# LuizGuzzo/Monocular_Depth_Estimation

Measured on AMD Instinct MI355X. Metric: training images/sec at 640x480 bs=32/GPU (GuideDepth, SSIM+0.1*L1, Adam), higher is better.
Workload: dtype fp32; 1 GPU; GuideDepth (DDRNet-23-slim + 3 guided upsampling blocks) train step, BASELINE cfg2, BN in train mode; global_batch=32, per_gpu_batch=32, resolution=640x480, parallelism=dp1

## Files before the change

### include/mde_abi.h

```cpp
#ifndef MDE_ABI_H
#define MDE_ABI_H

#include <stddef.h>
#include <stdint.h>

#ifdef __cplusplus
extern "C" {
#endif

#define MDE_ABI_VERSION 1

#define MDE_F32 0
#define MDE_BF16 1

#define MDE_OK 0
#define MDE_ERR_INVALID_ARG (-1)
#define MDE_ERR_UNSUPPORTED (-2)

int mde_abi_version(void);
const char* mde_status_string(int status);


int mde_bilinear_fwd(const void* x, void* y, int64_t n, int64_t c, int64_t hi,
                     int64_t wi, int64_t ho, int64_t wo, float scale_h,
// ... 234 lines not shown
int mde_conv3x3_wgrad(const void* gy, const void* x, float* gweight, int64_t n, int64_t cin,
                      int64_t cout, int64_t h, int64_t w, void* workspace, int dtype,
                      void* stream);

int mde_conv3x3s2_supported(int64_t cin, int64_t cout, int dtype);
size_t mde_conv3x3s2_wgrad_workspace(int64_t n, int64_t cin, int64_t cout, int64_t h, int64_t w,
                                     int dtype);
int mde_conv3x3s2_wgrad(const void* gy, const void* x, float* gweight, int64_t n, int64_t cin,
                        int64_t cout, int64_t h, int64_t w, void* workspace, int dtype,
                        void* stream);

size_t mde_dwconv_workspace(int64_t n, int64_t c, int64_t h, int64_t w, int64_t k,
                            int64_t stride, int64_t pad);
int mde_dwconv_fwd(const void* x, const float* weight, void* y, int64_t n, int64_t c,
                   int64_t h, int64_t w, int64_t k, int64_t stride, int64_t pad, int dtype,
                   void* stream);
int mde_dwconv_bwd(const void* gy, const void* x, const float* weight, void* gx,
                   float* gweight, int64_t n, int64_t c, int64_t h, int64_t w, int64_t k,
                   int64_t stride, int64_t pad, void* workspace, int dtype, void* stream);

size_t mde_layernorm_workspace(int64_t rows, int64_t c);
int mde_layernorm_fwd(const void* x, const float* gamma, const float* beta, void* y,
                      float* mean, float* rstd, int64_t rows, int64_t c, float eps, int dtype,
                      void* stream);
int mde_layernorm_bwd(const void* gy, const void* x, const float* gamma, const float* mean,
                      const float* rstd, void* gx, float* ggamma, float* gbeta, int64_t rows,
                      int64_t c, void* workspace, int dtype, void* stream);
int mde_layernorm_add_fwd(const void* x, const void* r, const float* gamma, const float* beta,
                          void* sum, void* y, float* mean, float* rstd, int64_t rows, int64_t c,
                          float eps, int dtype, void* stream);
int mde_layernorm_bwd_res(const void* gy, const void* x, const void* gres, const float* gamma,
                          const float* mean, const float* rstd, void* gx, float* ggamma,
                          float* gbeta, int64_t rows, int64_t c, void* workspace, int dtype,
                          void* stream);

int mde_transpose(const void* x, void* y, int64_t batch, int64_t m, int64_t n, int dtype,
                  void* stream);

int mde_nyu_augment(const void* image, const void* depth, const int32_t* flags, float* image_out,
                    float* depth_out, int64_t n, int64_t h, int64_t w, int64_t dh, int64_t dw,
                    int depth_bits, void* stream);

size_t mde_eval_workspace(int64_t n, int64_t h, int64_t w);
int mde_eval_sums(const void* pred, const void* gt, int64_t n, int64_t h, int64_t w,
                  float min_depth, float max_depth, int mode, const int32_t* crop,
                  void* workspace, double* sums, int dtype, void* stream);

int mde_conv3x3_guide_bf16_stats_blocks(int64_t n, int64_t cout, int64_t h, int64_t w);
int mde_conv3x3_guide_bf16_fwd(const float* x, const float* weight, void* y, float* stats,
                               int64_t n, int64_t cout, int64_t h, int64_t w, void* stream);

int mde_conv1x1_supported(int64_t cin, int64_t cout, int64_t h, int64_t w, int stride,
                          int dtype);
int mde_conv1x1_fwd(const void* x, const float* weight, void* y, int64_t n, int64_t cin,
                    int64_t cout, int64_t h, int64_t w, int stride, int dtype, void* stream);
int mde_conv1x1_bwd_data(const void* gy, const float* weight, void* gx, int64_t n, int64_t cin,
                         int64_t cout, int64_t h, int64_t w, int stride, int dtype,
                         void* stream);
size_t mde_conv1x1_wgrad_workspace(int64_t n, int64_t cin, int64_t cout, int64_t h, int64_t w,
                                   int stride, int dtype);
int mde_conv1x1_wgrad(const void* gy, const void* x, float* gweight, int64_t n, int64_t cin,
                      int64_t cout, int64_t h, int64_t w, int stride, void* workspace, int dtype,
                      void* stream);

int mde_conv3x3s2_fwd_supported(int64_t cin, int64_t cout, int64_t h, int64_t w, int dtype);
int mde_conv3x3s2_dgrad_supported(int64_t cin, int64_t cout, int64_t h, int64_t w, int dtype);
int mde_conv3x3s2_fwd(const void* x, const float* weight, void* y, int64_t n, int64_t cin,
                      int64_t cout, int64_t h, int64_t w, int dtype, void* stream);
int mde_conv3x3s2_bwd_data(const void* gy, const float* weight, void* gx, int64_t n, int64_t cin,
                           int64_t cout, int64_t h, int64_t w, int dtype, void* stream);

int mde_conv3x3_wide_supported(int64_t cin, int64_t cout, int64_t h, int64_t w, int pass,
                               int dtype);
int mde_conv3x3_wide_fwd(const void* x, const float* weight, void* y, int64_t n, int64_t cin,
                         int64_t cout, int64_t h, int64_t w, int dtype, void* stream);
int mde_conv3x3_wide_bwd_data(const void* gy, const float* weight, void* gx, int64_t n,
                              int64_t cin, int64_t cout, int64_t h, int64_t w, int dtype,
                              void* stream);

int mde_conv3x3s2_fwd_instance(int64_t n, int64_t cin, int64_t cout, int64_t h, int64_t w);
int mde_conv3x3s2_dgrad_instance(int64_t n, int64_t cin, int64_t cout, int64_t h, int64_t w);
int mde_conv3x3_wide_instance(int64_t n, int64_t cin, int64_t cout, int64_t h, int64_t w,
                              int pass);
int mde_conv3x3s2_instance_count(int which);

int mde_wino_mode(int mode);
int mde_wino_supported(int64_t cin, int64_t cout, int64_t h, int64_t w, int dtype);
size_t mde_wino_weight_bytes(int64_t cin, int64_t cout);
int mde_wino_weight(const float* weight, float* u, int64_t cin, int64_t cout, int flip,
                    void* stream);
int mde_wino_weight2(const float* weight, float* u, float* u_flip, int64_t cin, int64_t cout,
                     void* stream);
int mde_wino_conv(const float* x, const float* u, float* y, int64_t n, int64_t cin, int64_t cout,
                  int64_t h, int64_t w, int pass, int dtype, void* stream);
int mde_wino_conv_acc(const float* x, const float* u, const float* add, float* y, int64_t n,
                      int64_t cin, int64_t cout, int64_t h, int64_t w, int pass, int dtype,
                      void* stream);
int64_t mde_wino_weight_blocks(int64_t cin, int64_t cout, int both);
int mde_wino_weight_table(const int64_t* table, int rows, int64_t blocks, int64_t pairs,
                          void* stream);
int mde_wino_conv_stats(const float* x, const float* u, float* y, float* stats, int64_t n,
                        int64_t cin, int64_t cout, int64_t h, int64_t w, int pass, int dtype,
                        void* stream);
int mde_wino_stats_blocks(int64_t n, int64_t cin, int64_t cout, int64_t h, int64_t w);

int mde_graph_count_memsets(void* graph, int64_t* count);
// ... 88 lines not shown
```

### monocular_depth_estimation_amd/_abi.py

```python
from __future__ import annotations

import ctypes
import os

import torch

LIB_PATH = os.environ.get("MDE_HIP_LIB") or os.path.join(
    os.path.dirname(os.path.abspath(__file__)), "libmde_hip.so")

MDE_F32 = 0
MDE_BF16 = 1

_c = ctypes
_vp = _c.c_void_p
_i64 = _c.c_int64
_f32 = _c.c_float
_int = _c.c_int
_sz = _c.c_size_t
_fp = _c.POINTER(_c.c_float)

SIGNATURES = {
    "mde_abi_version": (_int, []),
    "mde_status_string": (_c.c_char_p, [_int]),
    "mde_bilinear_fwd": (_int, [_vp, _vp, _i64, _i64, _i64, _i64, _i64, _i64, _f32, _f32, _int, _int, _vp]),
# ... 70 lines not shown
                                            _vp, _vp, _vp, _i64, _i64, _i64, _i64, _vp, _i64, _vp,
                                            _int, _vp]),
    "mde_pointwise_bwd_bn": (_int, [_vp, _vp, _vp, _vp, _vp, _vp, _vp, _vp, _vp, _i64, _i64, _i64,
                                    _i64, _i64, _vp, _int, _vp]),
    "mde_pointwise_deferred_supported": (_int, [_i64, _i64, _i64, _i64]),
    "mde_pointwise_bwd_bn_deferred": (_int, [_vp, _i64, _i64, _vp, _vp, _vp, _vp, _vp, _vp, _vp, _vp,
                                             _vp, _vp, _vp, _vp, _i64, _i64, _i64, _i64, _i64, _vp,
                                             _int, _vp]),
    "mde_batchnorm_bwd_coef": (_int, [_vp, _vp, _vp, _vp, _int, _vp, _vp, _vp, _vp, _vp, _i64, _i64,
                                      _i64, _i64, _vp]),
    "mde_se_bn_bwd_coef": (_int, [_vp, _vp, _i64, _vp, _i64, _vp, _vp, _vp, _vp, _int, _vp, _vp, _i64,
                                  _vp, _vp, _vp, _vp, _vp, _vp, _vp, _vp, _vp, _i64, _i64, _i64, _vp,
                                  _int, _vp]),
    "mde_batchnorm_fwd_coef": (_int, [_vp, _vp, _vp, _vp, _vp, _vp, _vp, _f32, _f32, _int, _vp, _vp,
                                      _vp, _vp, _i64, _i64, _i64, _i64, _vp, _int, _vp]),
    "mde_conv3x3_supported": (_int, [_i64, _i64, _int, _int]),
    "mde_conv3x3_fwd": (_int, [_vp, _vp, _vp, _i64, _i64, _i64, _i64, _i64, _int, _vp]),
    "mde_conv3x3_bwd_data": (_int, [_vp, _vp, _vp, _i64, _i64, _i64, _i64, _i64, _int, _vp]),
    "mde_conv3x3_wgrad_workspace": (_sz, [_i64, _i64, _i64, _i64, _i64, _int]),
    "mde_conv3x3_wgrad": (_int, [_vp, _vp, _vp, _i64, _i64, _i64, _i64, _i64, _vp, _int, _vp]),
    "mde_conv3x3s2_supported": (_int, [_i64, _i64, _int]),
    "mde_conv3x3s2_wgrad_workspace": (_sz, [_i64, _i64, _i64, _i64, _i64, _int]),
    "mde_conv3x3s2_wgrad": (_int, [_vp, _vp, _vp, _i64, _i64, _i64, _i64, _i64, _vp, _int, _vp]),
    "mde_dwconv_workspace": (_sz, [_i64, _i64, _i64, _i64, _i64, _i64, _i64]),
    "mde_dwconv_fwd": (_int, [_vp, _vp, _vp, _i64, _i64, _i64, _i64, _i64, _i64, _i64, _int, _vp]),
    "mde_dwconv_bwd": (_int, [_vp, _vp, _vp, _vp, _vp, _i64, _i64, _i64, _i64, _i64, _i64, _i64,
                              _vp, _int, _vp]),
    "mde_layernorm_workspace": (_sz, [_i64, _i64]),
    "mde_layernorm_fwd": (_int, [_vp, _vp, _vp, _vp, _vp, _vp, _i64, _i64, _f32, _int, _vp]),
    "mde_layernorm_bwd": (_int, [_vp, _vp, _vp, _vp, _vp, _vp, _vp, _vp, _i64, _i64, _vp, _int,
                                 _vp]),
    "mde_layernorm_add_fwd": (_int, [_vp, _vp, _vp, _vp, _vp, _vp, _vp, _vp, _i64, _i64, _f32,
                                      _int, _vp]),
    "mde_layernorm_bwd_res": (_int, [_vp, _vp, _vp, _vp, _vp, _vp, _vp, _vp, _vp, _i64, _i64,
                                      _vp, _int, _vp]),
    "mde_transpose": (_int, [_vp, _vp, _i64, _i64, _i64, _int, _vp]),
    "mde_nyu_augment": (_int, [_vp, _vp, _vp, _vp, _vp, _i64, _i64, _i64, _i64, _i64, _int, _vp]),
    "mde_eval_workspace": (_sz, [_i64, _i64, _i64]),
    "mde_eval_sums": (_int, [_vp, _vp, _i64, _i64, _i64, _f32, _f32, _int, _c.POINTER(_c.c_int32), _vp,
                             _vp, _int, _vp]),
    "mde_colsum_workspace": (_sz, [_i64, _i64]),
    "mde_colsum": (_int, [_vp, _vp, _i64, _i64, _vp, _int, _vp]),
    "mde_head_conv_supported": (_int, [_i64, _i64, _i64, _i64]),
    "mde_head_conv_fwd": (_int, [_vp, _vp, _vp, _vp, _i64, _i64, _i64, _i64, _int, _vp]),
    "mde_head_conv_dgrad": (_int, [_vp, _vp, _vp, _i64, _i64, _i64, _i64, _int, _vp]),
    "mde_head_conv_wgrad_workspace": (_sz, [_i64, _i64, _i64, _i64]),
    "mde_head_conv_wgrad": (_int, [_vp, _vp, _vp, _i64, _i64, _i64, _i64, _vp, _int, _vp]),
    "mde_chansum_workspace": (_sz, [_i64, _i64, _i64]),
    "mde_chansum": (_int, [_vp, _vp, _i64, _i64, _i64, _vp, _int, _vp]),
    "mde_linear_wgrad_workspace": (_sz, [_i64, _i64, _i64]),
    "mde_linear_wgrad": (_int, [_vp, _vp, _vp, _vp, _i64, _i64, _i64, _vp, _int, _vp]),
    "mde_gelu_bwd_colsum": (_int, [_vp, _vp, _vp, _vp, _i64, _i64, _vp, _int, _vp]),
    "mde_conv1x1_supported": (_int, [_i64, _i64, _i64, _i64, _int, _int]),
    "mde_conv1x1_fwd": (_int, [_vp, _vp, _vp, _i64, _i64, _i64, _i64, _i64, _int, _int, _vp]),
    "mde_conv1x1_bwd_data": (_int, [_vp, _vp, _vp, _i64, _i64, _i64, _i64, _i64, _int, _int, _vp]),
    "mde_conv1x1_wgrad_workspace": (_sz, [_i64, _i64, _i64, _i64, _i64, _int, _int]),
    "mde_conv1x1_wgrad": (_int, [_vp, _vp, _vp, _i64, _i64, _i64, _i64, _i64, _int, _vp, _int,
                                 _vp]),
    "mde_conv3x3s2_fwd_supported": (_int, [_i64, _i64, _i64, _i64, _int]),
    "mde_conv3x3s2_dgrad_supported": (_int, [_i64, _i64, _i64, _i64, _int]),
    "mde_conv3x3s2_fwd": (_int, [_vp, _vp, _vp, _i64, _i64, _i64, _i64, _i64, _int, _vp]),
    "mde_conv3x3s2_bwd_data": (_int, [_vp, _vp, _vp, _i64, _i64, _i64, _i64, _i64, _int, _vp]),
    "mde_conv3x3_wide_supported": (_int, [_i64, _i64, _i64, _i64, _int, _int]),
    "mde_conv3x3_wide_fwd": (_int, [_vp, _vp, _vp, _i64, _i64, _i64, _i64, _i64, _int, _vp]),
    "mde_conv3x3_wide_bwd_data": (_int, [_vp, _vp, _vp, _i64, _i64, _i64, _i64, _i64, _int, _vp]),
    "mde_conv3x3s2_fwd_instance": (_int, [_i64, _i64, _i64, _i64, _i64]),
    "mde_conv3x3s2_dgrad_instance": (_int, [_i64, _i64, _i64, _i64, _i64]),
    "mde_conv3x3_wide_instance": (_int, [_i64, _i64, _i64, _i64, _i64, _int]),
    "mde_conv3x3s2_instance_count": (_int, [_int]),
    "mde_wino_mode": (_int, [_int]),
    "mde_wino_supported": (_int, [_i64, _i64, _i64, _i64, _int]),
    "mde_wino_weight_bytes": (_sz, [_i64, _i64]),
    "mde_wino_weight": (_int, [_vp, _vp, _i64, _i64, _int, _vp]),
    "mde_wino_weight2": (_int, [_vp, _vp, _vp, _i64, _i64, _vp]),
    "mde_wino_weight_blocks": (_i64, [_i64, _i64, _int]),
    "mde_wino_weight_table": (_int, [_vp, _int, _i64, _i64, _vp]),
    "mde_wino_conv": (_int, [_vp, _vp, _vp, _i64, _i64, _i64, _i64, _i64, _int, _int, _vp]),
    "mde_wino_conv_acc": (_int, [_vp, _vp, _vp, _vp, _i64, _i64, _i64, _i64, _i64, _int, _int, _vp]),
    "mde_wino_conv_stats": (_int, [_vp, _vp, _vp, _vp, _i64, _i64, _i64, _i64, _i64, _int, _int,
                                   _vp]),
    "mde_wino_stats_blocks": (_int, [_i64, _i64, _i64, _i64, _i64]),
    "mde_batchnorm_stats_route": (_int, [_i64, _i64, _i64, _i64, _i64, _int]),
    "mde_bn_chan_mode": (_int, [_int]),
    "mde_convbf_supported": (_int, [_i64, _i64, _i64, _i64, _int, _int, _int]),
    "mde_convbf_supported_n": (_int, [_i64, _i64, _i64, _i64, _i64, _int, _int, _int]),
    "mde_convbf_flops": (_c.c_double, [_i64, _i64, _i64, _i64, _i64, _int, _int, _int]),
    "mde_stem_bf16_supported": (_int, [_i64, _i64, _i64, _i64]),
    "mde_stem_bf16_fwd": (_int, [_vp, _vp, _vp, _i64, _i64, _i64, _i64, _vp]),
    "mde_stem_bf16_wgrad_workspace": (_sz, [_i64, _i64, _i64, _i64]),
    "mde_stem_bf16_wgrad": (_int, [_vp, _vp, _vp, _i64, _i64, _i64, _i64, _vp, _vp]),
    "mde_conv3x3_guide_bf16_wgrad_workspace": (_sz, [_i64, _i64, _i64, _i64]),
    "mde_conv3x3_guide_bf16_wgrad": (_int, [_vp, _vp, _vp, _i64, _i64, _i64, _i64, _vp, _vp]),
    "mde_convbf_pack_elems": (_sz, [_i64, _i64, _int, _int]),
    "mde_convbf_pack": (_int, [_vp, _vp, _i64, _i64, _int, _int, _vp]),
    "mde_convbf_pack_both": (_int, [_vp, _vp, _vp, _i64, _i64, _int, _vp]),
    "mde_convbf_pack_table": (_int, [_vp, _int, _i64, _i64, _vp]),
    "mde_convbf_stats_blocks": (_int, [_i64, _i64, _i64, _i64, _i64, _int, _int]),
    "mde_convbf_instance": (_int, [_i64, _i64, _i64, _i64, _i64, _int, _int, _int,
                                   _c.POINTER(_c.c_int32)]),
    "mde_convbf_instance_count": (_int, [_int]),
    "mde_convbf_fwd": (_int, [_vp, _vp, _vp, _vp, _i64, _i64, _i64, _i64, _i64, _int, _int, _vp]),
    "mde_convbf_bwd_data": (_int, [_vp, _vp, _vp, _i64, _i64, _i64, _i64, _i64, _int, _int, _vp]),
    "mde_convbf_wgrad_workspace": (_sz, [_i64, _i64, _i64, _i64, _i64, _int, _int]),
    "mde_convbf_wgrad": (_int, [_vp, _vp, _vp, _i64, _i64, _i64, _i64, _i64, _int, _int, _vp, _vp]),
    "mde_conv3x3_guide_bf16_stats_blocks": (_int, [_i64, _i64, _i64, _i64]),
    "mde_conv3x3_guide_bf16_fwd": (_int, [_vp, _vp, _vp, _vp, _i64, _i64, _i64, _i64, _vp]),
# ... 219 lines not shown
```

### monocular_depth_estimation_amd/csrc/conv1x1.hip

```cpp
#include <cstdlib>

#include "common.h"

namespace {

using f16v = float __attribute__((ext_vector_type(16)));

__device__ __forceinline__ f16v mfma32(float a, float b, f16v c) {
  return __builtin_amdgcn_mfma_f32_32x32x2f32(a, b, c, 0, 0, 0);
}

constexpr int KC = 32;
constexpr int KCP = 34;

__device__ __forceinline__ int xcd_logical(int total) {
  const int g = gridDim.x, per = g >> 3;
  const int b = blockIdx.x;
  const int l = (b & 7) * per + (b >> 3);
  return l < total ? l : -1;
}

inline unsigned xcd_grid(int64_t total) { return (unsigned)((total + 7) / 8 * 8); }

__device__ __forceinline__ int fdiv(int q, int d, float inv) {
// ... 91 lines not shown
      *reinterpret_cast<float4*>(sB + k * BQP + q) = rb[i];
    }
  };

  f16v acc[MT][QT];
#pragma unroll
  for (int a = 0; a < MT; ++a)
#pragma unroll
    for (int b = 0; b < QT; ++b)
#pragma unroll
      for (int r = 0; r < 16; ++r) acc[a][b][r] = 0.f;

  const float* pa = sA + (wm * 32 * MT + li) * KCP + h;
  const float* pb = sB + h * BQP + wq * 32 * QT + li;
  load(0);
  for (int k0 = 0; k0 < K; k0 += KC) {
    __syncthreads();
    store();
    __syncthreads();
    if (k0 + KC < K) load(k0 + KC);
#pragma unroll
    for (int s = 0; s < KC / 2; ++s) {
      float a[MT], b[QT];
#pragma unroll
      for (int x = 0; x < MT; ++x) a[x] = pa[x * 32 * KCP + 2 * s];
#pragma unroll
      for (int y = 0; y < QT; ++y) b[y] = pb[2 * s * BQP + y * 32];
#pragma unroll
      for (int x = 0; x < MT; ++x)
#pragma unroll
        for (int y = 0; y < QT; ++y) acc[x][y] = mfma32(a[x], b[y], acc[x][y]);
    }
  }

  float* ob = out + (int64_t)img * M * hout * wout;
#pragma unroll
  for (int y = 0; y < QT; ++y) {
    const int q = q0 + wq * 32 * QT + 32 * y + li;
    if (q >= Q) continue;
    int64_t po = q;
    int rr = 0, cc = 0;
    if constexpr (SOUT == 2) {
      rr = fdiv(q, wo, inv_wo);
      cc = q - rr * wo;
      po = (int64_t)(2 * rr) * wout + 2 * cc;
    }
#pragma unroll
    for (int x = 0; x < MT; ++x)
#pragma unroll
      for (int r = 0; r < 16; ++r) {
        const int m = m0 + wm * 32 * MT + 32 * x + (r & 3) + 8 * (r >> 2) + 4 * h;
        if (PAD && m >= M) continue;
        float* dst = ob + (int64_t)m * hout * wout + po;
        if constexpr (SOUT == 1) {
          *dst = acc[x][y][r];
        } else {
          *reinterpret_cast<float2*>(dst) = make_float2(acc[x][y][r], 0.f);
          if (2 * rr + 1 < hout) *reinterpret_cast<float2*>(dst + wout) = make_float2(0.f, 0.f);
        }
      }
  }
}

template <int BCO, int BCI, int MT, int NT, int SIN>
__global__ void __launch_bounds__(256)
    c1_wgrad_kernel(const float* __restrict__ gy, const float* __restrict__ x,
                    float* __restrict__ part, int CO, int CI, int Q, int hin, int win, int wo,
                    int64_t npix, int nchunks, int ksplit, int cotiles, int citiles, int total) {
  constexpr int WN = BCI / (32 * NT), WMv = BCO / (32 * MT);
  static_assert(WN * WMv == 4, "four waves per block");
  constexpr int AV = BCO * KC / 1024, BV = BCI * KC / 1024;
  static_assert(AV >= 1 && BV >= 1, "tile too small");
  __shared__ __attribute__((aligned(16))) float sA[BCO * KCP];
  __shared__ __attribute__((aligned(16))) float sB[BCI * KCP];
  const int lb = xcd_logical(total);
  if (lb < 0) return;
  const int ntile = cotiles * citiles;
  const int tile = lb % ntile, ks = lb / ntile;
  const int cot = tile % cotiles, cit = tile / cotiles;
  const int co0 = cot * BCO, ci0 = cit * BCI;
  const int c_begin = (int)((int64_t)nchunks * ks / ksplit);
  const int c_end = (int)((int64_t)nchunks * (ks + 1) / ksplit);
  const int tid = threadIdx.x, lane = tid & 63, li = lane & 31, h = lane >> 5;
  const int wv = __builtin_amdgcn_readfirstlane(tid >> 6);
  const int wm = wv / WN, wn = wv % WN;
  const int64_t hwin = (int64_t)hin * win;

  const float inv_wo = 1.f / (float)wo;
  float4 ra[AV], rb[BV];
  auto load = [&](int chunk) {
    const int p0 = chunk * KC;
    const int n0 = p0 / Q, q0 = p0 - n0 * Q;
#pragma unroll
    for (int i = 0; i < AV; ++i) {
      const int e = 4 * (tid + 256 * i);
      const int row = e / KC, k = e % KC;
      const bool wrap = q0 + k >= Q;
      const int n = n0 + (wrap ? 1 : 0), q = q0 + k - (wrap ? Q : 0);
      const bool ok = p0 + k < npix && co0 + row < CO;
      const int cr = co0 + row < CO ? co0 + row : CO - 1;
      const float4 t = *reinterpret_cast<const float4*>(
          gy + ((ok ? n : 0) * CO + cr) * Q + (ok ? q : 0));
      ra[i] = ok ? t : make_float4(0.f, 0.f, 0.f, 0.f);
    }
#pragma unroll
    for (int i = 0; i < BV; ++i) {
// ... 331 lines not shown
  static const bool on = [] {
    const char* e = std::getenv("MDE_C1_SMALL");
    return !(e && e[0] == '0');
  }();
  return on;
}

inline bool small_plan(int64_t n, int64_t ci, int64_t co, int64_t q, SmallWg* p) {
  if (!c1_small_on() || q % 16) return false;
  if (ci % 32 == 0 && co % 32 == 0) return false;
  const int co16 = (int)mde::cdiv(co, 16), ci16 = (int)mde::cdiv(ci, 16);
  if (co16 * ci16 > 24) return false;
  int bm = 0, bn = 0, best = 1 << 30;
  for (int mt : {1, 2, 4, 8})
    for (int nt : {1, 2, 4, 8}) {
      if (mt * nt > 8) continue;
      const int g = (int)(mde::cdiv(co16, mt) * mde::cdiv(ci16, nt));
      const int waste = g * mt * nt;
      if (g <= 3 && waste < best) {
        best = waste;
        bm = mt;
        bn = nt;
      }
    }
  if (!bm) return false;
  p->mt = bm;
  p->nt = bn;
  p->groups_ci = (int)mde::cdiv(ci16, bn);
  p->groups = (int)mde::cdiv(co16, bm) * p->groups_ci;
  p->nchunks = n * q / 16;
  int64_t blocks = 512 / p->groups;
  if (blocks > p->nchunks / 4) blocks = p->nchunks / 4 > 1 ? p->nchunks / 4 : 1;
  p->per_block = mde::cdiv(p->nchunks, blocks);
  p->blocks = mde::cdiv(p->nchunks, p->per_block);
  return true;
}

inline size_t small_ws_bytes(const SmallWg& p, int64_t ci, int64_t co) {
  return sizeof(float) * (size_t)(p.blocks * ci * co);
}

inline bool c1_shape_ok(int64_t n, int64_t ci, int64_t co, int64_t h, int64_t w, int stride) {
  if (n <= 0 || h <= 0 || w <= 0 || (stride != 1 && stride != 2)) return false;
  if (ci % 8 || co % 8 || ci < 16 || co < 16) return false;
  const int64_t ho = (h - 1) / stride + 1, wo = (w - 1) / stride + 1;
  if ((ho * wo) % 4) return false;
  if (stride == 2 && w % 2) return false;
  return n * ci * h * w < (int64_t)1 << 31 && n * co * ho * wo < (int64_t)1 << 31 &&
         ho * wo >= KC && ho < (1 << 12) && wo < (1 << 10);
}

inline int cm_bm(int64_t m) { return m % 128 == 0 ? 128 : (m % 64 == 0 ? 64 : 32); }

template <int SIN, int SOUT, bool TRANSA>
int launch_cm(const float* in, const float* wt, float* out, int64_t n, int64_t K, int64_t M,
              int64_t hin, int64_t win, int64_t ho, int64_t wo, int64_t hout, int64_t wout,
              int kid, double bytes, double flops, hipStream_t s) {
  const int64_t Q = ho * wo;
  const int bm = cm_bm(M);
  constexpr int BQ = 128;
  const int64_t qtiles = mde::cdiv(Q, BQ), mtiles = mde::cdiv(M, bm);
  const int64_t total = n * qtiles * mtiles;
  if (total > 0x7fffffff) return MDE_ERR_INVALID_ARG;
  const dim3 grid(xcd_grid(total)), block(256);
  const bool pad = K % KC || M % bm;
#define MDE_CM(BMv, MTv, QTv)                                                                     \
  do {                                                                                            \
    if (pad)                                                                                      \
      MDE_LAUNCH_MFMA(kid, bytes, flops, s,                                                       \
                      (cm_kernel<BMv, BQ, MTv, QTv, SIN, SOUT, TRANSA, true>), grid, block, 0,    \
                      in, wt, out, (int)K, (int)M, (int)hin, (int)win, (int)wo, (int)Q,           \
                      (int)hout, (int)wout, (int)qtiles, (int)mtiles, (int)total);                \
    else                                                                                          \
      MDE_LAUNCH_MFMA(kid, bytes, flops, s, (cm_kernel<BMv, BQ, MTv, QTv, SIN, SOUT, TRANSA>),    \
                      grid, block, 0, in, wt, out, (int)K, (int)M, (int)hin, (int)win, (int)wo,   \
                      (int)Q, (int)hout, (int)wout, (int)qtiles, (int)mtiles, (int)total);        \
  } while (0)
  if (bm == 128)
    MDE_CM(128, 2, 2);
  else if (bm == 64)
    MDE_CM(64, 2, 1);
  else
    MDE_CM(32, 1, 1);
#undef MDE_CM
  return MDE_OK;
}

struct WgPlan {
  int bco, bci, cotiles, citiles, ksplit, nchunks;
  int64_t npix;
};

inline WgPlan wg_plan(int64_t n, int64_t ci, int64_t co, int64_t ho, int64_t wo) {
  WgPlan p;
  const int a = co % 128 == 0 ? 128 : (co % 64 == 0 ? 64 : 32);
  const int b = ci % 128 == 0 ? 128 : (ci % 64 == 0 ? 64 : 32);
  if (b == 32) {
    p.bco = 128;
    p.bci = 32;
  } else if (a == 32) {
    p.bco = 32;
    p.bci = 128;
  } else {
    p.bco = a;
    p.bci = b;
  }
  p.cotiles = (int)mde::cdiv(co, p.bco);
  p.citiles = (int)mde::cdiv(ci, p.bci);
  p.npix = n * ho * wo;
  p.nchunks = (int)mde::cdiv(p.npix, KC);
  const int tiles = p.cotiles * p.citiles;
  int ks = (int)mde::cdiv(512, tiles);
  if (ks > p.nchunks / 8) ks = p.nchunks / 8;
  const int64_t cap = ((int64_t)16 << 20) / (ci * co);
  if (ks > cap) ks = (int)cap;
  p.ksplit = ks < 1 ? 1 : ks;
  return p;
}

}

extern "C" {

int mde_conv1x1_supported(int64_t cin, int64_t cout, int64_t h, int64_t w, int stride,
                          int dtype) {
  return dtype == MDE_F32 && c1_shape_ok(1, cin, cout, h, w, stride) ? 1 : 0;
}

int mde_conv1x1_fwd(const void* x, const float* weight, void* y, int64_t n, int64_t cin,
                    int64_t cout, int64_t h, int64_t w, int stride, int dtype, void* stream) {
  if (dtype != MDE_F32) return MDE_ERR_UNSUPPORTED;
  if (!x || !weight || !y) return MDE_ERR_INVALID_ARG;
  if (!c1_shape_ok(n, cin, cout, h, w, stride)) return MDE_ERR_UNSUPPORTED;
  hipStream_t s = (hipStream_t)stream;
  const int64_t ho = (h - 1) / stride + 1, wo = (w - 1) / stride + 1;
  const double flops = 2.0 * n * ho * wo * (double)cin * cout;
  const double bytes = 4.0 * n * (double)ho * wo * (cin + cout);
  if (stride == 1) {
    if (const int mt = mix_small_mt(cout, cin))
      return launch_mix_small<false>(mt, (const float*)x, weight, (float*)y, n, cin, cout, ho * wo,
                                     mde::K_C1_FWD, bytes, flops, s);
    return launch_cm<1, 1, false>((const float*)x, weight, (float*)y, n, cin, cout, h, w, ho, wo,
                                  ho, wo, mde::K_C1_FWD, bytes, flops, s);
  }
  return launch_cm<2, 1, false>((const float*)x, weight, (float*)y, n, cin, cout, h, w, ho, wo,
                                ho, wo, mde::K_C1_FWD, bytes, flops, s);
}

int mde_conv1x1_bwd_data(const void* gy, const float* weight, void* gx, int64_t n, int64_t cin,
                         int64_t cout, int64_t h, int64_t w, int stride, int dtype,
                         void* stream) {
  if (dtype != MDE_F32) return MDE_ERR_UNSUPPORTED;
  if (!gy || !weight || !gx) return MDE_ERR_INVALID_ARG;
  if (!c1_shape_ok(n, cin, cout, h, w, stride)) return MDE_ERR_UNSUPPORTED;
  hipStream_t s = (hipStream_t)stream;
  const int64_t ho = (h - 1) / stride + 1, wo = (w - 1) / stride + 1;
  const double flops = 2.0 * n * ho * wo * (double)cin * cout;
  const double bytes = 4.0 * n * ((double)ho * wo * cout + (double)h * w * cin);
  if (stride == 1) {
    if (const int mt = mix_small_mt(cin, cout))
      return launch_mix_small<true>(mt, (const float*)gy, weight, (float*)gx, n, cout, cin, ho * wo,
                                    mde::K_C1_DGRAD, bytes, flops, s);
    return launch_cm<1, 1, true>((const float*)gy, weight, (float*)gx, n, cout, cin, ho, wo, ho,
                                 wo, h, w, mde::K_C1_DGRAD, bytes, flops, s);
  }
  return launch_cm<1, 2, true>((const float*)gy, weight, (float*)gx, n, cout, cin, ho, wo, ho, wo,
                               h, w, mde::K_C1_DGRAD, bytes, flops, s);
}

size_t mde_conv1x1_wgrad_workspace(int64_t n, int64_t cin, int64_t cout, int64_t h, int64_t w,
                                   int stride, int dtype) {
  if (dtype != MDE_F32 || !c1_shape_ok(n, cin, cout, h, w, stride)) return 0;
  const int64_t ho = (h - 1) / stride + 1, wo = (w - 1) / stride + 1;
  SmallWg sp;
  if (stride == 1 && small_plan(n, cin, cout, ho * wo, &sp)) return small_ws_bytes(sp, cin, cout);
  const WgPlan p = wg_plan(n, cin, cout, ho, wo);
  return sizeof(float) * (size_t)p.ksplit * (size_t)(cin * cout);
}

// ... 70 lines not shown
```

### monocular_depth_estimation_amd/nn.py

```python
from __future__ import annotations

import contextlib
import os

import torch
from torch import nn

from . import _abi
from .functional import GradSlot, _amp_bwd, _amp_fwd, _gpu, _ws

_ACTS = {"none": 0, "relu": 1, "hardswish": 2}


_bn_fwd = torch.amp.custom_fwd(device_type="cuda")


class _BatchNormAct(torch.autograd.Function):
    @staticmethod
    @_bn_fwd
    def forward(ctx, x, weight, bias, prebias, residual, running_mean, running_var, nbt,
                training, momentum, eps, act, stats=None, res_slot=None):
        dt = torch.bfloat16 if x.dtype == torch.bfloat16 else torch.float32
        x = x.to(dt).contiguous()
        residual = residual.to(dt).contiguous() if residual is not None else None
# ... 652 lines not shown
        weight = weight.contiguous()
        ctx.save_for_backward(x, weight)
        n, cin, h, w = x.shape
        cout = weight.shape[0]
        if S2_FWD and _abi.query("mde_conv3x3s2_fwd_supported", cin, cout, h, w, _abi.MDE_F32):
            y = torch.empty((n, cout, (h - 1) // 2 + 1, (w - 1) // 2 + 1), dtype=x.dtype,
                            device=x.device)
            _abi.call("mde_conv3x3s2_fwd", _abi.ptr(x), _abi.ptr(weight), _abi.ptr(y), n, cin, cout,
                      h, w, _abi.dtype_code(x), _abi.stream_of(x))
            return y
        return torch.nn.functional.conv2d(x, weight, None, 2, 1)

    @staticmethod
    def backward(ctx, gy):
        x, weight = ctx.saved_tensors
        gy = gy.contiguous()
        n, cin, h, w = x.shape
        cout = weight.shape[0]
        gx = gw = None
        if ctx.needs_input_grad[0]:
            if S2_FWD and _abi.query("mde_conv3x3s2_dgrad_supported", cin, cout, h, w,
                                     _abi.MDE_F32):
                gx = torch.empty_like(x)
                _abi.call("mde_conv3x3s2_bwd_data", _abi.ptr(gy), _abi.ptr(weight), _abi.ptr(gx), n,
                          cin, cout, h, w, _abi.dtype_code(gy), _abi.stream_of(gy))
            else:
                gx = torch.ops.aten.convolution_backward(
                    gy, x, weight, None, (2, 2), (1, 1), (1, 1), False, (0, 0), 1,
                    (True, False, False))[0]
        if ctx.needs_input_grad[1]:
            nws = _abi.query("mde_conv3x3s2_wgrad_workspace", n, cin, cout, h, w, _abi.MDE_F32) \
                if (S2_WGRAD and (S2_WIDE or cout == 32)
                    and _abi.query("mde_conv3x3s2_supported", cin, cout, _abi.MDE_F32)) else 0
            if nws > 0:
                gw = torch.empty_like(weight)
                _abi.call("mde_conv3x3s2_wgrad", _abi.ptr(gy), _abi.ptr(x), _abi.ptr(gw), n, cin,
                          cout, h, w, _abi.ptr(_ws(nws, x)), _abi.MDE_F32, _abi.stream_of(gy))
            else:
                gw = torch.ops.aten.convolution_backward(
                    gy, x, weight, None, (2, 2), (1, 1), (1, 1), False, (0, 0), 1,
                    (False, True, False))[1]
        return gx, gw


class _Conv1x1(torch.autograd.Function):

    @staticmethod
    def forward(ctx, x, weight, stride):
        x = x.contiguous()
        weight = weight.contiguous()
        ctx.save_for_backward(x, weight)
        ctx.stride = stride
        cin, cout = x.shape[1], weight.shape[0]
        if stride == 1 and not (C1_FWD == "all" or (C1_FWD == "pad" and (cin % 32 or cout % 32))):
            return torch.nn.functional.conv2d(x, weight)
        n, cin, h, w = x.shape
        cout = weight.shape[0]
        ho, wo = (h - 1) // stride + 1, (w - 1) // stride + 1
        y = torch.empty((n, cout, ho, wo), dtype=x.dtype, device=x.device)
        _abi.call("mde_conv1x1_fwd", _abi.ptr(x), _abi.ptr(weight), _abi.ptr(y), n, cin, cout, h, w,
                  stride, _abi.dtype_code(x), _abi.stream_of(x))
        return y

    @staticmethod
    def backward(ctx, gy):
        x, weight = ctx.saved_tensors
        gy = gy.contiguous()
        n, cin, h, w = x.shape
        cout = weight.shape[0]
        st = _abi.stream_of(gy)
        gx = gw = None
        if ctx.needs_input_grad[0]:
            gx = torch.empty_like(x)
            _abi.call("mde_conv1x1_bwd_data", _abi.ptr(gy), _abi.ptr(weight), _abi.ptr(gx), n, cin,
                      cout, h, w, ctx.stride, _abi.dtype_code(gy), st)
        if ctx.needs_input_grad[1]:
            gw = torch.empty_like(weight)
            ws = _ws(_abi.query("mde_conv1x1_wgrad_workspace", n, cin, cout, h, w, ctx.stride,
                                _abi.MDE_F32), x)
            _abi.call("mde_conv1x1_wgrad", _abi.ptr(gy), _abi.ptr(x), _abi.ptr(gw), n, cin, cout, h,
                      w, ctx.stride, _abi.ptr(ws), _abi.dtype_code(gy), st)
        return gx, gw, None


C1_WIDE = os.environ.get("MDE_C1_WIDE", "1") != "0"
C1_PAD = os.environ.get("MDE_C1_PAD", "1") != "0"
C1_FWD = os.environ.get("MDE_C1_FWD", "pad")


def conv1x1_ok(conv: nn.Conv2d, x) -> bool:
    if not (C1_WIDE and x.is_cuda and x.dtype == torch.float32 and not _autocast_bf16(x)
            and conv.weight.dtype == torch.float32 and x.dim() == 4
            and conv.kernel_size == (1, 1) and conv.padding == (0, 0)
            and conv.dilation == (1, 1) and conv.groups == 1
            and conv.stride in ((1, 1), (2, 2)) and conv.padding_mode == "zeros"):
        return False
    if not C1_PAD and (conv.in_channels % 32 or conv.out_channels % 32):
        return False
    return bool(_abi.query("mde_conv1x1_supported", conv.in_channels, conv.out_channels,
                           x.shape[2], x.shape[3], conv.stride[0], _abi.MDE_F32))


def conv3x3s2_ok(conv: nn.Conv2d, x) -> bool:
    if not (x.is_cuda and x.dtype == torch.float32 and not _autocast_bf16(x)
            and conv.weight.dtype == torch.float32 and x.dim() == 4 and x.shape[-1] % 2 == 0
            and conv.kernel_size == (3, 3) and conv.stride == (2, 2) and conv.padding == (1, 1)
            and conv.dilation == (1, 1) and conv.groups == 1 and conv.padding_mode == "zeros"):
        return False
    cin, cout, h, w = conv.in_channels, conv.out_channels, x.shape[2], x.shape[3]
    wgrad = (S2_WGRAD and bool(_abi.query("mde_conv3x3s2_supported", cin, cout, _abi.MDE_F32))
             and (S2_WIDE or cout == 32)
             and _abi.query("mde_conv3x3s2_wgrad_workspace", x.shape[0], cin, cout, h, w,
                            _abi.MDE_F32) > 0)
    fwd = S2_FWD and bool(_abi.query("mde_conv3x3s2_fwd_supported", cin, cout, h, w, _abi.MDE_F32))
    return wgrad or fwd


S2_WGRAD = os.environ.get("MDE_S2_WGRAD", "1") != "0"
S2_FWD = os.environ.get("MDE_S2_FWD", "1") != "0"
S2_WIDE = os.environ.get("MDE_S2_WIDE", "1") != "0"


def conv3x3_passes(conv: nn.Conv2d, x):
    if (conv.kernel_size != (3, 3) or conv.stride != (1, 1) or conv.padding != (1, 1)
            or conv.dilation != (1, 1) or conv.groups != 1 or conv.padding_mode != "zeros"
            or x.dim() != 4 or conv.weight.dtype != torch.float32):
        return None
    cin, cout = conv.in_channels, conv.out_channels
    if _conv3x3_bf16_path(cin, cout, x, conv.weight):
        p, dt = CONV3X3_HIP_BF16[(cin, cout)], _abi.MDE_BF16
    elif x.dtype == torch.float32:
        p, dt = CONV3X3_HIP.get((cin, cout), (False, False, False)), _abi.MDE_F32
    else:
        return None
    p = [bool(f) and bool(_abi.query("mde_conv3x3_supported", cin, cout, i, dt))
         for i, f in enumerate(p)]
    if (dt == _abi.MDE_F32 and WIDE_WGRAD_ALL and not p[2] and cout % 64 == 0
            and _abi.query("mde_conv3x3_supported", cin, cout, 2, dt)
            and (cin % 32 == 0 or (WIDE_PAD and _abi.query(
                "mde_conv3x3_wgrad_workspace", x.shape[0], cin, cout, x.shape[2], x.shape[3],
# ... 848 lines not shown
```

Measured before the change: 1047 images/s.

## Add flattened batch-pixel tiling for small-spatial 1x1 convs and widen wgrad split

Adds a cmf_kernel that tiles the 1x1 conv GEMM over the flattened batch*pixel dimension instead of per image, picking a tile shape with a cost model so small-resolution layers fill all CUs. Wgrad planning shrinks tiles and raises the K-split when too few blocks would launch. The forward path also now routes aligned stride-1 1x1 convs to the HIP kernel when the batch has enough pixels, instead of to the library conv. Risks include losing library conv efficiency on some shapes and extra atomic/reduction work from the larger wgrad split.

```diff
diff --git a/include/mde_abi.h b/include/mde_abi.h
--- a/include/mde_abi.h
+++ b/include/mde_abi.h
@@ -310,6 +310,16 @@
 
 int mde_conv1x1_supported(int64_t cin, int64_t cout, int64_t h, int64_t w, int stride,
                           int dtype);
+#define MDE_C1_I_FWD_BLOCKS 0
+#define MDE_C1_I_DGRAD_BLOCKS 1
+#define MDE_C1_I_WGRAD_BLOCKS 2
+#define MDE_C1_I_WGRAD_SLABS 3
+#define MDE_C1_I_CUS 4
+#define MDE_C1_I_FWD_TILE 5
+#define MDE_C1_I_DGRAD_TILE 6
+#define MDE_C1_I_WGRAD_TILE 7
+int64_t mde_conv1x1_instance(int64_t n, int64_t cin, int64_t cout, int64_t h, int64_t w, int stride,
+                         int what);
 int mde_conv1x1_fwd(const void* x, const float* weight, void* y, int64_t n, int64_t cin,
                     int64_t cout, int64_t h, int64_t w, int stride, int dtype, void* stream);
 int mde_conv1x1_bwd_data(const void* gy, const float* weight, void* gx, int64_t n, int64_t cin,
diff --git a/monocular_depth_estimation_amd/_abi.py b/monocular_depth_estimation_amd/_abi.py
--- a/monocular_depth_estimation_amd/_abi.py
+++ b/monocular_depth_estimation_amd/_abi.py
@@ -146,6 +146,7 @@
     "mde_linear_wgrad": (_int, [_vp, _vp, _vp, _vp, _i64, _i64, _i64, _vp, _int, _vp]),
     "mde_gelu_bwd_colsum": (_int, [_vp, _vp, _vp, _vp, _i64, _i64, _vp, _int, _vp]),
     "mde_conv1x1_supported": (_int, [_i64, _i64, _i64, _i64, _int, _int]),
+    "mde_conv1x1_instance": (_i64, [_i64, _i64, _i64, _i64, _i64, _int, _int]),
     "mde_conv1x1_fwd": (_int, [_vp, _vp, _vp, _i64, _i64, _i64, _i64, _i64, _int, _int, _vp]),
     "mde_conv1x1_bwd_data": (_int, [_vp, _vp, _vp, _i64, _i64, _i64, _i64, _i64, _int, _int, _vp]),
     "mde_conv1x1_wgrad_workspace": (_sz, [_i64, _i64, _i64, _i64, _i64, _int, _int]),
diff --git a/monocular_depth_estimation_amd/csrc/conv1x1.hip b/monocular_depth_estimation_amd/csrc/conv1x1.hip
--- a/monocular_depth_estimation_amd/csrc/conv1x1.hip
+++ b/monocular_depth_estimation_amd/csrc/conv1x1.hip
@@ -167,6 +167,172 @@
         const int m = m0 + wm * 32 * MT + 32 * x + (r & 3) + 8 * (r >> 2) + 4 * h;
         if (PAD && m >= M) continue;
         float* dst = ob + (int64_t)m * hout * wout + po;
+        if constexpr (SOUT == 1) {
+          *dst = acc[x][y][r];
+        } else {
+          *reinterpret_cast<float2*>(dst) = make_float2(acc[x][y][r], 0.f);
+          if (2 * rr + 1 < hout) *reinterpret_cast<float2*>(dst + wout) = make_float2(0.f, 0.f);
+        }
+      }
+  }
+}
+
+template <int BM, int BQ, int MT, int QT, int SIN, int SOUT, bool TRANSA, bool PAD>
+__global__ void __launch_bounds__(64 * (BM / (32 * MT)) * (BQ / (32 * QT)))
+    cmf_kernel(const float* __restrict__ in, const float* __restrict__ wt, float* __restrict__ out,
+               int K, int M, int hin, int win, int wo, int Q, int hout, int wout, int NP,
+               int mtiles, int total) {
+  constexpr int WQ = BQ / (32 * QT), WM = BM / (32 * MT), NT = 64 * WQ * WM;
+  static_assert(NT == 64 || NT == 128 || NT == 256, "one, two or four waves per block");
+  constexpr int BQP = BQ + 32;
+  constexpr int AV = BM * KC / (4 * NT);
+  constexpr int BV = KC * BQ / (4 * NT);
+  static_assert(AV >= 1 && BV >= 1, "tile too small");
+  constexpr int BE = SIN == 1 ? 1 : 4;
+  __shared__ __attribute__((aligned(16))) float sA[BM * KCP];
+  __shared__ __attribute__((aligned(16))) float sB[KC * BQP];
+
+  const int lb = xcd_logical(total);
+  if (lb < 0) return;
+  const int mt = lb % mtiles, jt = lb / mtiles;
+  const int m0 = mt * BM, j0 = jt * BQ;
+  const int tid = threadIdx.x, lane = tid & 63, li = lane & 31, h = lane >> 5;
+  const int wv = __builtin_amdgcn_readfirstlane(tid >> 6);
+  const int wm = wv / WQ, wq = wv % WQ;
+  const int hwin = hin * win;
+  const float inv_wo = 1.f / (float)wo;
+
+  int bo[BV][BE];
+#pragma unroll
+  for (int i = 0; i < BV; ++i) {
+    const int jc = j0 + (4 * (tid + NT * i)) % BQ;
+    const bool ok = jc < NP;
+    const int img = ok ? jc / Q : 0, q = jc - img * Q;
+    const int base = img * K * hwin;
+    if constexpr (SIN == 1) {
+      bo[i][0] = ok ? base + q : -1;
+    } else {
+#pragma unroll
+      for (int j = 0; j < 4; ++j) {
+        const int qq = ok ? q + j : 0, r = fdiv(qq, wo, inv_wo), c = qq - r * wo;
+        bo[i][j] = ok ? base + 2 * r * win + 2 * c : -1;
+      }
+    }
+  }
+
+  float4 ra[AV], rb[BV];
+  auto load = [&](int k0) {
+#pragma unroll
+    for (int i = 0; i < AV; ++i) {
+      const int e = 4 * (tid + NT * i);
+      if constexpr (TRANSA) {
+        const int k = e / BM, m = e % BM;
+        const bool ok = !PAD || (k0 + k < K && m0 + m < M);
+        const float4 t = *reinterpret_cast<const float4*>(wt + (ok ? (int64_t)(k0 + k) * M + m0 + m : 0));
+        ra[i] = ok ? t : make_float4(0.f, 0.f, 0.f, 0.f);
+      } else {
+        const int m = e / KC, k = e % KC;
+        const bool ok = !PAD || (k0 + k < K && m0 + m < M);
+        const float4 t = *reinterpret_cast<const float4*>(wt + (ok ? (int64_t)(m0 + m) * K + k0 + k : 0));
+        ra[i] = ok ? t : make_float4(0.f, 0.f, 0.f, 0.f);
+      }
+    }
+#pragma unroll
+    for (int i = 0; i < BV; ++i) {
+      const int k = (4 * (tid + NT * i)) / BQ;
+      const bool kok = !PAD || k0 + k < K;
+      const float* src = in + (kok ? k0 + k : 0) * hwin;
+      if constexpr (SIN == 1) {
+        const bool ok = kok && bo[i][0] >= 0;
+        const float4 t = *reinterpret_cast<const float4*>(src + (ok ? bo[i][0] : 0));
+        rb[i] = ok ? t : make_float4(0.f, 0.f, 0.f, 0.f);
+      } else {
+        float v[4];
+#pragma unroll
+        for (int j = 0; j < 4; ++j) {
+          const bool ok = kok && bo[i][j] >= 0;
+          const float t = src[ok ? bo[i][j] : 0];
+          v[j] = ok ? t : 0.f;
+        }
+        rb[i] = make_float4(v[0], v[1], v[2], v[3]);
+      }
+    }
+  };
+  auto store = [&]() {
+#pragma unroll
+    for (int i = 0; i < AV; ++i) {
+      const int e = 4 * (tid + NT * i);
+      if constexpr (TRANSA) {
+        const int k = e / BM, m = e % BM;
+        sA[(m + 0) * KCP + k] = ra[i].x;
+        sA[(m + 1) * KCP + k] = ra[i].y;
+        sA[(m + 2) * KCP + k] = ra[i].z;
+        sA[(m + 3) * KCP + k] = ra[i].w;
+      } else {
+        const int m = e / KC, k = e % KC;
+        *reinterpret_cast<float2*>(sA + m * KCP + k) = make_float2(ra[i].x, ra[i].y);
+        *reinterpret_cast<float2*>(sA + m * KCP + k + 2) = make_float2(ra[i].z, ra[i].w);
+      }
+    }
+#pragma unroll
+    for (int i = 0; i < BV; ++i) {
+      const int e = 4 * (tid + NT * i);
+      const int k = e / BQ, q = e % BQ;
+      *reinterpret_cast<float4*>(sB + k * BQP + q) = rb[i];
+    }
+  };
+
+  f16v acc[MT][QT];
+#pragma unroll
+  for (int a = 0; a < MT; ++a)
+#pragma unroll
+    for (int b = 0; b < QT; ++b)
+#pragma unroll
+      for (int r = 0; r < 16; ++r) acc[a][b][r] = 0.f;
+
+  const float* pa = sA + (wm * 32 * MT + li) * KCP + h;
+  const float* pb = sB + h * BQP + wq * 32 * QT + li;
+  load(0);
+  for (int k0 = 0; k0 < K; k0 += KC) {
+    __syncthreads();
+    store();
+    __syncthreads();
+    if (k0 + KC < K) load(k0 + KC);
+#pragma unroll
+    for (int s = 0; s < KC / 2; ++s) {
+      float a[MT], b[QT];
+#pragma unroll
+      for (int x = 0; x < MT; ++x) a[x] = pa[x * 32 * KCP + 2 * s];
+#pragma unroll
+      for (int y = 0; y < QT; ++y) b[y] = pb[2 * s * BQP + y * 32];
+#pragma unroll
+      for (int x = 0; x < MT; ++x)
+#pragma unroll
+        for (int y = 0; y < QT; ++y) acc[x][y] = mfma32(a[x], b[y], acc[x][y]);
+    }
+  }
+
+  const int64_t hwout = (int64_t)hout * wout;
+#pragma unroll
+  for (int y = 0; y < QT; ++y) {
+    const int jj = j0 + wq * 32 * QT + 32 * y + li;
+    if (jj >= NP) continue;
+    const int img = jj / Q, q = jj - img * Q;
+    int64_t po = q;
+    int rr = 0, cc = 0;
+    if constexpr (SOUT == 2) {
+      rr = fdiv(q, wo, inv_wo);
+      cc = q - rr * wo;
+      po = (int64_t)(2 * rr) * wout + 2 * cc;
+    }
+    float* ob = out + (int64_t)img * M * hwout + po;
+#pragma unroll
+    for (int x = 0; x < MT; ++x)
+#pragma unroll
+      for (int r = 0; r < 16; ++r) {
+        const int m = m0 + wm * 32 * MT + 32 * x + (r & 3) + 8 * (r >> 2) + 4 * h;
+        if (PAD && m >= M) continue;
+        float* dst = ob + (int64_t)m * hwout;
         if constexpr (SOUT == 1) {
           *dst = acc[x][y][r];
         } else {
@@ -604,16 +770,102 @@
 
 inline int cm_bm(int64_t m) { return m % 128 == 0 ? 128 : (m % 64 == 0 ? 64 : 32); }
 
+inline bool c1_flat_on() {
+  static const bool on = [] {
+    const char* e = std::getenv("MDE_C1_FLAT");
+    return !(e && e[0] == '0');
+  }();
+  return on;
+}
+
+constexpr int C1_CUS = 256;
+constexpr int C1_SIMDS = 4 * C1_CUS;
+constexpr int64_t C1_FLAT_Q = 4800;
+
+struct CmPlan {
+  int flat, bm, bq, mt, qt;
+  int64_t mtiles, qtiles, total;
+};
+
+inline CmPlan cm_plan(int64_t n, int64_t M, int64_t Q) {
+  CmPlan p;
+  p.flat = 0;
+  p.bm = cm_bm(M);
+  p.bq = 128;
+  p.mt = p.qt = 0;
+  p.mtiles = mde::cdiv(M, p.bm);
+  p.qtiles = mde::cdiv(Q, 128);
+  p.total = n * p.qtiles * p.mtiles;
+  if (!c1_flat_on() || Q >= C1_FLAT_Q) return p;
+  static const int cand[5][4] = {{128, 128, 2, 2}, {64, 64, 1, 1}, {32, 128, 1, 1},
+                                 {32, 64, 1, 1}, {32, 32, 1, 1}};
+  const int64_t np = n * Q;
+  int64_t best_cost = 0, best_blocks = 0;
+  for (const auto& c : cand) {
+    if (c[0] > cm_bm(M)) continue;
+    const int64_t mtiles = mde::cdiv(M, c[0]), qtiles = mde::cdiv(np, c[1]);
+    const int64_t blocks = mtiles * qtiles;
+    const int64_t waves = blocks * (c[0] / (32 * c[2])) * (c[1] / (32 * c[3]));
+    const int64_t cost = mde::cdiv(waves, C1_SIMDS) * c[2] * c[3];
+    const bool take = !p.flat || cost * 8 <= best_cost * 7 ||
+                      (best_blocks < C1_CUS && blocks > best_blocks && cost <= best_cost);
+    if (!take) continue;
+    best_cost = cost;
+    best_blocks = blocks;
+    p.flat = 1;
+    p.bm = c[0];
+    p.bq = c[1];
+    p.mt = c[2];
+    p.qt = c[3];
+    p.mtiles = mtiles;
+    p.qtiles = qtiles;
+    p.total = blocks;
+  }
+  return p;
+}
+
 template <int SIN, int SOUT, bool TRANSA>
 int launch_cm(const float* in, const float* wt, float* out, int64_t n, int64_t K, int64_t M,
               int64_t hin, int64_t win, int64_t ho, int64_t wo, int64_t hout, int64_t wout,
               int kid, double bytes, double flops, hipStream_t s) {
   const int64_t Q = ho * wo;
-  const int bm = cm_bm(M);
+  const CmPlan pl = cm_plan(n, M, Q);
+  if (pl.total > 0x7fffffff) return MDE_ERR_INVALID_ARG;
+  if (pl.flat) {
+    const dim3 fgrid(xcd_grid(pl.total));
+    const bool fpad = K % KC || M % pl.bm;
+#define MDE_CMF(BMv, BQv, MTv, QTv)                                                                \
+  do {                                                                                             \
+    if (fpad)                                                                                      \
+      MDE_LAUNCH_MFMA(kid, bytes, flops, s,                                                        \
+                      (cmf_kernel<BMv, BQv, MTv, QTv, SIN, SOUT, TRANSA, true>), fgrid,            \
+                      dim3(64 * (BMv / (32 * MTv)) * (BQv / (32 * QTv))), 0, in, wt, out, (int)K,  \
+                      (int)M, (int)hin, (int)win, (int)wo, (int)Q, (int)hout, (int)wout,           \
+                      (int)(n * Q), (int)pl.mtiles, (int)pl.total);                                \
+    else                                                                                           \
+      MDE_LAUNCH_MFMA(kid, bytes, flops, s,                                                        \
+                      (cmf_kernel<BMv, BQv, MTv, QTv, SIN, SOUT, TRANSA, false>), fgrid,           \
+                      dim3(64 * (BMv / (32 * MTv)) * (BQv / (32 * QTv))), 0, in, wt, out, (int)K,  \
+                      (int)M, (int)hin, (int)win, (int)wo, (int)Q, (int)hout, (int)wout,           \
+                      (int)(n * Q), (int)pl.mtiles, (int)pl.total);                                \
+  } while (0)
+    if (pl.bm == 128)
+      MDE_CMF(128, 128, 2, 2);
+    else if (pl.bm == 64)
+      MDE_CMF(64, 64, 1, 1);
+    else if (pl.bq == 128)
+      MDE_CMF(32, 128, 1, 1);
+    else if (pl.bq == 64)
+      MDE_CMF(32, 64, 1, 1);
+    else
+      MDE_CMF(32, 32, 1, 1);
+#undef MDE_CMF
+    return MDE_OK;
+  }
+  const int bm = pl.bm;
   constexpr int BQ = 128;
-  const int64_t qtiles = mde::cdiv(Q, BQ), mtiles = mde::cdiv(M, bm);
-  const int64_t total = n * qtiles * mtiles;
-  if (total > 0x7fffffff) return MDE_ERR_INVALID_ARG;
+  const int64_t qtiles = pl.qtiles, mtiles = pl.mtiles;
+  const int64_t total = pl.total;
   const dim3 grid(xcd_grid(total)), block(256);
   const bool pad = K % KC || M % bm;
 #define MDE_CM(BMv, MTv, QTv)                                                                     \
@@ -661,12 +913,24 @@
   p.citiles = (int)mde::cdiv(ci, p.bci);
   p.npix = n * ho * wo;
   p.nchunks = (int)mde::cdiv(p.npix, KC);
-  const int tiles = p.cotiles * p.citiles;
-  int ks = (int)mde::cdiv(512, tiles);
-  if (ks > p.nchunks / 8) ks = p.nchunks / 8;
+  int tiles = p.cotiles * p.citiles;
   const int64_t cap = ((int64_t)16 << 20) / (ci * co);
-  if (ks > cap) ks = (int)cap;
-  p.ksplit = ks < 1 ? 1 : ks;
+  auto split = [&](int blocks, int minchunks) {
+    int ks = (int)mde::cdiv(blocks, tiles);
+    if (ks > p.nchunks / minchunks) ks = p.nchunks / minchunks;
+    if (ks > cap) ks = (int)cap;
+    return ks < 1 ? 1 : ks;
+  };
+  p.ksplit = split(512, 8);
+  if (!c1_flat_on() || tiles * p.ksplit >= C1_CUS) return p;
+  if (p.bco == 128 && p.bci != 32) p.bco = 64;
+  if (p.bci == 128 && p.bco != 32) p.bci = 64;
+  p.cotiles = (int)mde::cdiv(co, p.bco);
+  p.citiles = (int)mde::cdiv(ci, p.bci);
+  tiles = p.cotiles * p.citiles;
+  p.ksplit = split(512, 8);
+  for (int minchunks = 4; tiles * p.ksplit < C1_CUS && minchunks >= 2; minchunks /= 2)
+    p.ksplit = split(C1_CUS, minchunks);
   return p;
 }
 
@@ -677,6 +941,41 @@
 int mde_conv1x1_supported(int64_t cin, int64_t cout, int64_t h, int64_t w, int stride,
                           int dtype) {
   return dtype == MDE_F32 && c1_shape_ok(1, cin, cout, h, w, stride) ? 1 : 0;
+}
+
+int64_t mde_conv1x1_instance(int64_t n, int64_t cin, int64_t cout, int64_t h, int64_t w, int stride,
+                         int what) {
+  if (what == MDE_C1_I_CUS) return C1_CUS;
+  if (!c1_shape_ok(n, cin, cout, h, w, stride)) return -1;
+  const int64_t ho = (h - 1) / stride + 1, wo = (w - 1) / stride + 1, Q = ho * wo;
+  switch (what) {
+    case MDE_C1_I_FWD_BLOCKS:
+    case MDE_C1_I_FWD_TILE:
+    case MDE_C1_I_DGRAD_BLOCKS:
+    case MDE_C1_I_DGRAD_TILE: {
+      const bool fwd = what == MDE_C1_I_FWD_BLOCKS || what == MDE_C1_I_FWD_TILE;
+      const bool tile = what == MDE_C1_I_FWD_TILE || what == MDE_C1_I_DGRAD_TILE;
+      const int64_t M = fwd ? cout : cin, K = fwd ? cin : cout;
+      if (stride == 1 && mix_small_mt(M, K)) return tile ? 0 : mde::cdiv(n * mde::cdiv(Q, 64), 4);
+      const CmPlan p = cm_plan(n, M, Q);
+      return tile ? p.flat * 1000000 + p.bm * 1000 + p.bq : p.total;
+    }
+    case MDE_C1_I_WGRAD_BLOCKS:
+    case MDE_C1_I_WGRAD_SLABS:
+    case MDE_C1_I_WGRAD_TILE: {
+      SmallWg sp;
+      if (stride == 1 && small_plan(n, cin, cout, Q, &sp))
+        return what == MDE_C1_I_WGRAD_BLOCKS  ? sp.blocks * sp.groups
+               : what == MDE_C1_I_WGRAD_SLABS ? sp.blocks
+                                                 : 0;
+      const WgPlan p = wg_plan(n, cin, cout, ho, wo);
+      return what == MDE_C1_I_WGRAD_BLOCKS  ? (int64_t)p.cotiles * p.citiles * p.ksplit
+             : what == MDE_C1_I_WGRAD_SLABS ? p.ksplit
+                                               : p.bco * 1000 + p.bci;
+    }
+    default:
+      return -1;
+  }
 }
 
 int mde_conv1x1_fwd(const void* x, const float* weight, void* y, int64_t n, int64_t cin,
diff --git a/monocular_depth_estimation_amd/nn.py b/monocular_depth_estimation_amd/nn.py
--- a/monocular_depth_estimation_amd/nn.py
+++ b/monocular_depth_estimation_amd/nn.py
@@ -728,7 +728,7 @@
         ctx.save_for_backward(x, weight)
         ctx.stride = stride
         cin, cout = x.shape[1], weight.shape[0]
-        if stride == 1 and not (C1_FWD == "all" or (C1_FWD == "pad" and (cin % 32 or cout % 32))):
+        if stride == 1 and not _c1_fwd_hip(x.shape[0], cin, cout, x.shape[2] * x.shape[3]):
             return torch.nn.functional.conv2d(x, weight)
         n, cin, h, w = x.shape
         cout = weight.shape[0]
@@ -761,7 +761,19 @@
 
 C1_WIDE = os.environ.get("MDE_C1_WIDE", "1") != "0"
 C1_PAD = os.environ.get("MDE_C1_PAD", "1") != "0"
-C1_FWD = os.environ.get("MDE_C1_FWD", "pad")
+C1_FWD = os.environ.get("MDE_C1_FWD", "auto")
+C1_FLAT = os.environ.get("MDE_C1_FLAT", "1") != "0"
+C1_FWD_PIXELS = 32768
+
+
+def _c1_fwd_hip(n, cin, cout, pixels) -> bool:
+    if C1_FWD == "all":
+        return True
+    if C1_FWD == "none":
+        return False
+    if cin % 32 or cout % 32:
+        return True
+    return C1_FWD == "auto" and C1_FLAT and n * pixels >= C1_FWD_PIXELS
 
 
 def conv1x1_ok(conv: nn.Conv2d, x) -> bool:
```

After: 1055 images/s (median of 6 runs). About the same (+0.8%).
